# jc-bao/gym-xarm

Hardware: AMD Instinct MI355X
Metric: env steps/sec (whole node), XarmPDPickAndPlace-v0 (higher is better)
Workload: dtype f32

## Files before the change

gym_xarm_amd/build.py:

```python
import os
import shutil
import subprocess
import sys

HERE = os.path.dirname(os.path.abspath(__file__))
CSRC = os.path.join(HERE, "csrc")
LIB = os.path.join(CSRC, "libxarm_hip.so")
UNITS = ["xarm_hip.hip", "xarm_k_pnp.hip", "xarm_k_pnp_coop.hip", "xarm_k_reach.hip", "xarm_k_handover.hip", "xarm_k_handover_coop.hip",
         "xarm_k_handover2.hip", "xarm_k_stack.hip", "xarm_k_rearrange.hip", "xarm_k_render.hip", "xarm_k_her.hip", "xarm_k_norm.hip", "xarm_k_policy.hip"]
HEADERS = ["xarm_dev.h", "xarm_core.h", "xarm7_pd_model.h", "xarm_reach_core.h", "xarm7_reach_model.h", "xarm_handover_core.h", "xarm_handover2_core.h",
           "xarm_stack_core.h", "xarm_rearrange_core.h", "xarm_cubes_dev.h", "xarm_coop_core.h", "xarm_reach_coop_core.h", "xarm_handover_coop_core.h", "xarm_render_core.h",
           "xarm_render_model.h", "xarm_her_core.h", "xarm_norm_core.h", "xarm_policy_core.h"]
SOURCES = UNITS + HEADERS
UNIT_FLAGS = {"xarm_k_handover_coop.hip": ["-ffp-contract=on", "-DXC_SWEEP_COPY", "-DXC_PAD_ROWS_V1", "-DXC_PAD_SETUP_V1"], "xarm_k_norm.hip": ["-ffp-contract=off"],
              "xarm_k_policy.hip": ["-ffp-contract=off"]}
_SCHED = [] if os.environ.get("XARM_SCHED", "ilp") == "default" else ["-mllvm", "-amdgpu-sched-strategy=iterative-ilp"]
HIPCC_FLAGS = ["--offload-arch=gfx950", "-O3", "-std=c++17", "-fPIC", "-Wno-unused-value", "-fno-slp-vectorize"] + _SCHED

def find_hipcc():
    for c in (os.environ.get("HIPCC"), shutil.which("hipcc"), "/opt/rocm/bin/hipcc"):
        if c and os.path.exists(c):
            return c
    raise RuntimeError("hipcc not found (need ROCm); set HIPCC=/path/to/hipcc")


def stale():
    if not os.path.exists(LIB):
        return True
    deps = [os.path.join(CSRC, s) for s in SOURCES] + [os.path.join(os.path.dirname(HERE), "include", "xarm_hip.h")]
    t = os.path.getmtime(LIB)
    return any(os.path.getmtime(d) > t for d in deps if os.path.exists(d))


def _compile(args):
    cmd, verbose = args
    if verbose:
        print(" ".join(cmd), flush=True)
    subprocess.check_call(cmd)


def build(force=False, verbose=True, extra_flags=(), lib=LIB, jobs=None):
    from concurrent.futures import ThreadPoolExecutor
    for g in ("gen_model_header.py", "gen_render_header.py"):
        gen = os.path.join(os.path.dirname(HERE), "tools", g)
        if os.path.exists(gen):
            subprocess.check_call([sys.executable, gen], stdout=subprocess.DEVNULL)
    if not force and lib == LIB and not stale():
        return lib
    hipcc = find_hipcc()
    objdir = os.path.join(CSRC, "build" if lib == LIB else "build_" + os.path.splitext(os.path.basename(lib))[0])
    os.makedirs(objdir, exist_ok=True)
    objs, jobs_l = [], []
    for u in UNITS:
        o = os.path.join(objdir, os.path.splitext(u)[0] + ".o")
        objs.append(o)
        jobs_l.append(([hipcc] + HIPCC_FLAGS + UNIT_FLAGS.get(u, []) + list(extra_flags) + ["-c", "-o", o, os.path.join(CSRC, u)], verbose))
    with ThreadPoolExecutor(jobs or min(len(UNITS), os.cpu_count() or 1)) as ex:
        list(ex.map(_compile, jobs_l))
    _compile(([hipcc, "--offload-arch=gfx950", "-shared", "-fPIC", "-o", lib] + objs, verbose))
    return lib


def build_example(verbose=True):
    root = os.path.dirname(HERE)
    src, out = os.path.join(root, "examples", "abi_step_loop.c"), os.path.join(root, "examples", "abi_step_loop")
    if not os.path.exists(src):
        return None
    if os.path.exists(out) and os.path.getmtime(out) >= max(os.path.getmtime(src), os.path.getmtime(os.path.join(root, "include", "xarm_hip.h"))):
        return out
    rocm = os.environ.get("ROCM_PATH", "/opt/rocm")
    cmd = ["gcc", "-O2", "-std=c11", "-I", os.path.join(root, "include"), "-I", os.path.join(rocm, "include"), src,
           "-L", CSRC, "-lxarm_hip", "-L", os.path.join(rocm, "lib"), "-lamdhip64",
           "-Wl,-rpath,$ORIGIN/../gym_xarm_amd/csrc", "-Wl,-rpath," + os.path.join(rocm, "lib"), "-o", out]
    if verbose:
        print(" ".join(cmd), flush=True)
    subprocess.check_call(cmd)
    return out


if __name__ == "__main__":
    build(force="--force" in sys.argv)
    print(LIB)
```

gym_xarm_amd/csrc/xarm_coop_core.h:

```cpp
#pragma once
#include "xarm_core.h"

namespace xc {
using xk::V3; using xk::mk; using xk::dot; using xk::cross; using xk::symmul; using xk::tri; using xk::symi;
using xk::EnvState; using xk::EnvCfg; using xk::NTS; using xk::NP; using xk::clampT; using xk::xabs; using xk::xsqrt;
using xk::LDS_S; using xk::LDS_T;

constexpr int GL = 16;
constexpr int NT = 3 * NTS;
constexpr int NA1 = 14;
constexpr int NF = 3 * NP;
constexpr int NLA = 7;
constexpr int C0_T = 0, C0_F = NT, C0_N = NT + NF;
constexpr int C1_A = 0, C1_L = NA1, C1_F = NA1 + NLA, C1_N = NA1 + NLA + NF;
constexpr int C2_T = 0, C2_A = NT, C2_L = NT + NA1, C2_F = NT + NA1 + NLA, C2_N = NT + NA1 + NLA + NF;

#if defined(__HIPCC__) && !defined(XARM_HOST_BUILD)
constexpr int LVN = 1;
struct Grp { int l; };
XARM_HD int lane_of(const Grp &G, int) { return G.l; }
template <int CTRL> XARM_HD float dpp(float x) {
    return __builtin_bit_cast(float, __builtin_amdgcn_update_dpp(0, __builtin_bit_cast(int, x), CTRL, 0xf, 0xf, true));
}
#else
// ... 39 lines not shown
template <typename T> XARM_HD LV<T> lv_med3(LV<T> x, LV<T> lo, LV<T> hi) { LV<T> r; XC_LANES r.v[i_] = med3(x.v[i_], lo.v[i_], hi.v[i_]); return r; }
XARM_HD float max0(float x) { return __builtin_fmaxf(x, 0.0f); }
XARM_HD double max0(double x) { return x < 0.0 ? 0.0 : x; }
template <typename T> XARM_HD LV<T> lv_max0(LV<T> x) { LV<T> r; XC_LANES r.v[i_] = max0(x.v[i_]); return r; }
template <int L, typename T> XARM_HD void lv_commit(const Grp &G, LV<T> &dst, LV<T> src) {
    XC_LANES dst.v[i_] = lane_of(G, i_) == L ? src.v[i_] : dst.v[i_];
}
#if defined(__HIPCC__) && !defined(XARM_HOST_BUILD)
template <int L> XARM_HD LV<float> lv_bcast(LV<float> x) { LV<float> r; r.v[0] = dpp<0x150 + L>(x.v[0]); return r; }
XARM_HD float lv_allsum(LV<float> x) {
    XC_NO_CONTRACT
    float s = x.v[0];
    s += dpp<0xB1>(s);
    s += dpp<0x4E>(s);
    s += dpp<0x141>(s);
    s += dpp<0x140>(s);
    return s;
}
#else
template <int L, typename T> XARM_HD LV<T> lv_bcast(LV<T> x) { LV<T> r; XC_LANES r.v[i_] = x.v[L]; return r; }
template <typename T> XARM_HD T lv_allsum(LV<T> x) {
    T a[GL], b[GL];
    for (int i = 0; i < GL; i++) a[i] = x.v[i];
    for (int i = 0; i < GL; i++) b[i] = a[i] + a[i ^ 1];
    for (int i = 0; i < GL; i++) a[i] = b[i] + b[i ^ 2];
    for (int i = 0; i < GL; i++) b[i] = a[i] + a[(i & 8) | (7 - (i & 7))];
    for (int i = 0; i < GL; i++) a[i] = b[i] + b[15 - i];
    return a[0];
}
#endif
template <int L, typename T> XARM_HD T lv_get(LV<T> x) { return lv_bcast<L>(x).v[0]; }
#if defined(__HIPCC__) && !defined(XARM_HOST_BUILD)
XARM_HD LV<float> lv_suffix_sum(LV<float> x) {
    XC_NO_CONTRACT
    float s = x.v[0];
    s += dpp<0x101>(s);
    s += dpp<0x102>(s);
    s += dpp<0x104>(s);
    s += dpp<0x108>(s);
    LV<float> r; r.v[0] = s; return r;
}
#else
template <typename T> XARM_HD LV<T> lv_suffix_sum(LV<T> x) {
    T a[GL], b[GL];
    for (int i = 0; i < GL; i++) a[i] = x.v[i];
    for (int sh = 1; sh < GL; sh *= 2) {
        for (int i = 0; i < GL; i++) b[i] = a[i] + (i + sh < GL ? a[i + sh] : (T)0);
        for (int i = 0; i < GL; i++) a[i] = b[i];
    }
    LV<T> r; for (int i = 0; i < GL; i++) r.v[i] = a[i]; return r;
}
#endif

#if defined(__HIPCC__) && !defined(XARM_HOST_BUILD)
template <typename T> struct LV2 { xk::xf2 v; };
XARM_HD LV2<float> lv2_make(LV<float> x, LV<float> y) { LV2<float> r; r.v.x = x.v[0]; r.v.y = y.v[0]; return r; }
XARM_HD LV<float> lv2_x(LV2<float> a) { LV<float> r; r.v[0] = a.v.x; return r; }
XARM_HD LV<float> lv2_y(LV2<float> a) { LV<float> r; r.v[0] = a.v.y; return r; }
XARM_HD LV2<float> lv2_fma(LV2<float> a, LV2<float> b, LV2<float> c) { LV2<float> r; r.v = __builtin_elementwise_fma(a.v, b.v, c.v); return r; }
XARM_HD LV2<float> lv2_sub(LV2<float> a, LV2<float> b) { XC_NO_CONTRACT LV2<float> r; r.v = a.v - b.v; return r; }
XARM_HD LV2<float> lv2_mul(LV2<float> a, LV2<float> b) { XC_NO_CONTRACT LV2<float> r; r.v = a.v * b.v; return r; }
template <int L> XARM_HD void lv2_commit(const Grp &G, LV2<float> &dst, LV2<float> src) { dst.v = G.l == L ? src.v : dst.v; }
template <int L> XARM_HD LV2<float> lv2_bcast(LV2<float> x) {
    LV2<float> r;
    const long long in = __builtin_bit_cast(long long, x.v);
    const long long out = __builtin_amdgcn_update_dpp(0ll, in, 0x150 + L, 0xf, 0xf, true);
    r.v = __builtin_bit_cast(xk::xf2, out);
    return r;
}
#else
template <typename T> struct LV2 { LV<T> x, y; };
template <typename T> XARM_HD LV2<T> lv2_make(LV<T> x, LV<T> y) { LV2<T> r; r.x = x; r.y = y; return r; }
template <typename T> XARM_HD LV<T> lv2_x(LV2<T> a) { return a.x; }
template <typename T> XARM_HD LV<T> lv2_y(LV2<T> a) { return a.y; }
template <typename T> XARM_HD LV2<T> lv2_fma(LV2<T> a, LV2<T> b, LV2<T> c) { return lv2_make(lv_fma(a.x, b.x, c.x), lv_fma(a.y, b.y, c.y)); }
template <typename T> XARM_HD LV2<T> lv2_sub(LV2<T> a, LV2<T> b) { return lv2_make(lv_sub(a.x, b.x), lv_sub(a.y, b.y)); }
template <typename T> XARM_HD LV2<T> lv2_mul(LV2<T> a, LV2<T> b) { return lv2_make(lv_mul(a.x, b.x), lv_mul(a.y, b.y)); }
template <int L, typename T> XARM_HD void lv2_commit(const Grp &G, LV2<T> &dst, LV2<T> src) { lv_commit<L>(G, dst.x, src.x); lv_commit<L>(G, dst.y, src.y); }
template <int L, typename T> XARM_HD LV2<T> lv2_bcast(LV2<T> x) { return lv2_make(lv_bcast<L>(x.x), lv_bcast<L>(x.y)); }
#endif

template <typename T> XARM_HD T sel3(int k, T a, T b, T c) { return k == 0 ? a : (k == 1 ? b : c); }
template <typename T> XARM_HD T sel4(int k, T a, T b, T c, T d) { return k == 0 ? a : (k == 1 ? b : (k == 2 ? c : d)); }
template <typename T> XARM_HD V3<T> selv3(int k, V3<T> a, V3<T> b, V3<T> c) { return mk<T>(sel3(k, a.x, b.x, c.x), sel3(k, a.y, b.y, c.y), sel3(k, a.z, b.z, c.z)); }
template <typename T> XARM_HD V3<T> selv4(int k, V3<T> a, V3<T> b, V3<T> c, V3<T> d) {
    return mk<T>(sel4(k, a.x, b.x, c.x, d.x), sel4(k, a.y, b.y, c.y, d.y), sel4(k, a.z, b.z, c.z, d.z));
}

template <typename T> struct Setup {
    T Minv[45], dq[9];
    V3<T> hc1;
    V3<T> cb, vb, wb;
    T Iinv[6];
    V3<T> tr[NTS];
    T tvt[NTS], tl0[NTS];
    int tid[NTS];
    T m_vt[9], la_vt[7], la_sg[7], lf_vt[2][2], g_vt;
    LV<T> lpp[3], lpn[3], lpt1[3], lpvt, lpl0;
    bool pact[NP];
    bool pad_any, la_any;
    T pad_cfm, mu_p;
};

enum { R_J0 = 0,
       R_J1 = 6,
       R_J2A = 15,
       R_J2B = 24,
       R_J3 = 30,
       R_G = 37,
       R_L0 = 41,
       R_LO1 = 45, R_HI1 = 46,
       R_CFM = 47,
       R_N = 48 };

template <typename T> XARM_HD V3<T> tdir(int a) { return mk<T>(a == 2 ? (T)1 : (T)0, a == 1 ? (T)-1 : (T)0, a == 0 ? (T)1 : (T)0); }

template <typename T, typename Scene = xk::PnpScene>
XARM_HD void lane_rows_base(const Setup<T> &S, int l, T (&R)[R_N]) {
    const T inf = (T)3.0e38;
#pragma unroll
    for (int k = 0; k < R_N; k++) R[k] = (T)0;
    {
        const int s = l / 3, a = l - 3 * s;
        const bool own = l < NT;
        const V3<T> d = tdir<T>(a);
        const V3<T> r = selv4(s, S.tr[0], S.tr[1], S.tr[2], S.tr[3]);
        const V3<T> rd = cross(r, d);
        R[R_J0 + 0] = own ? d.x : (T)0; R[R_J0 + 1] = own ? d.y : (T)0; R[R_J0 + 2] = own ? d.z : (T)0;
        R[R_J0 + 3] = own ? rd.x : (T)0; R[R_J0 + 4] = own ? rd.y : (T)0; R[R_J0 + 5] = own ? rd.z : (T)0;
        const T vt = a == 0 ? sel4(s, S.tvt[0], S.tvt[1], S.tvt[2], S.tvt[3]) : (T)0;
        const T ju = R[R_J0 + 0] * S.vb.x + R[R_J0 + 1] * S.vb.y + R[R_J0 + 2] * S.vb.z + R[R_J0 + 3] * S.wb.x + R[R_J0 + 4] * S.wb.y + R[R_J0 + 5] * S.wb.z;
        R[R_G + 0] = own ? vt - ju : (T)0;
        R[R_L0 + 0] = (own && a == 0) ? sel4(s, S.tl0[0], S.tl0[1], S.tl0[2], S.tl0[3]) : (T)0;
    }
    {
#pragma unroll
        for (int d = 0; d < 7; d++) R[R_J1 + d] = l == d ? (T)1 : (T)0;
        R[R_J1 + 7] = (l == 7 || l == 9 || l == 13) ? (T)1 : (l == 10 ? (T)-1 : (T)0);
        R[R_J1 + 8] = (l == 8 || l == 11) ? (T)1 : ((l == 12 || l == 13) ? (T)-1 : (T)0);
        T vt = (T)0, ju = (T)0;
#pragma unroll
        for (int d = 0; d < 9; d++) { vt = l == d ? S.m_vt[d] : vt; ju += R[R_J1 + d] * S.dq[d]; }
        vt = l == 9 ? S.lf_vt[0][0] : (l == 10 ? S.lf_vt[0][1] : (l == 11 ? S.lf_vt[1][0] : (l == 12 ? S.lf_vt[1][1] : (l == 13 ? S.g_vt : vt))));
        R[R_G + 1] = l < NA1 ? vt - ju : (T)0;
        const T m_hi_arm = (T)(xm::ARM_MOTOR_FORCE * Scene::TIME_STEP), m_hi_fin = (T)(Scene::FINGER_MOTOR_FORCE * Scene::TIME_STEP);
        const T g_hi = (T)(xm::GEAR_MAX_FORCE * Scene::TIME_STEP);
        const T hi = l < 7 ? m_hi_arm : (l < 9 ? m_hi_fin : (l < 13 ? inf : (l == 13 ? g_hi : (T)0)));
        R[R_HI1] = hi;
        R[R_LO1] = (l >= 9 && l < 13) ? (T)0 : -hi;
    }
}

template <typename T, typename Lds, bool PAD, bool LA>
XARM_HD void lane_rows_extra(const Setup<T> &S, Lds lds, int l, int li, T (&R)[R_N]) {
    if (PAD) {
        const int idx = l / 3, a = l - 3 * idx;
        const bool own = l < NF;
        const int fk = idx / xm::NPAD;
        const V3<T> p = mk<T>(S.lpp[0].v[li], S.lpp[1].v[li], S.lpp[2].v[li]);
        const V3<T> n = mk<T>(S.lpn[0].v[li], S.lpn[1].v[li], S.lpn[2].v[li]);
        const V3<T> t1 = mk<T>(S.lpt1[0].v[li], S.lpt1[1].v[li], S.lpt1[2].v[li]);
        const V3<T> t2 = cross(n, t1);
        const V3<T> d = selv3(a, n, t1, t2);
        const V3<T> mo = cross(p, d);
        const V3<T> af = S.hc1 * (fk == 0 ? (T)1 : (T)-1);
        const T wf = dot(af, d);
        T ju = (T)0;
#pragma unroll
        for (int i = 0; i < 7; i++) {
            const T j = lds[LDS_S + i * 6 + 0] * mo.x + lds[LDS_S + i * 6 + 1] * mo.y + lds[LDS_S + i * 6 + 2] * mo.z +
                        lds[LDS_S + i * 6 + 3] * d.x + lds[LDS_S + i * 6 + 4] * d.y + lds[LDS_S + i * 6 + 5] * d.z;
            R[R_J2A + i] = own ? j : (T)0;
            ju += R[R_J2A + i] * S.dq[i];
        }
        R[R_J2A + 7] = (own && fk == 0) ? wf : (T)0;
        R[R_J2A + 8] = (own && fk == 1) ? wf : (T)0;
        ju += R[R_J2A + 7] * S.dq[7] + R[R_J2A + 8] * S.dq[8];
        const V3<T> rb = p - S.cb;
        const V3<T> rd = cross(rb, d);
        R[R_J2B + 0] = own ? -d.x : (T)0; R[R_J2B + 1] = own ? -d.y : (T)0; R[R_J2B + 2] = own ? -d.z : (T)0;
        R[R_J2B + 3] = own ? -rd.x : (T)0; R[R_J2B + 4] = own ? -rd.y : (T)0; R[R_J2B + 5] = own ? -rd.z : (T)0;
        ju += R[R_J2B + 0] * S.vb.x + R[R_J2B + 1] * S.vb.y + R[R_J2B + 2] * S.vb.z + R[R_J2B + 3] * S.wb.x + R[R_J2B + 4] * S.wb.y + R[R_J2B + 5] * S.wb.z;
        const T vt = a == 0 ? S.lpvt.v[li] : (T)0;
        R[R_G + 2] = own ? vt - ju : (T)0;
        R[R_L0 + 2] = (own && a == 0) ? S.lpl0.v[li] : (T)0;
        R[R_CFM] = (own && a == 0) ? S.pad_cfm : (T)0;
    }
    if (LA) {
        T vt = (T)0, ju = (T)0;
#pragma unroll
        for (int d = 0; d < 7; d++) {
            R[R_J3 + d] = l == d ? S.la_sg[d] : (T)0;
            vt = l == d ? S.la_vt[d] : vt;
            ju += R[R_J3 + d] * S.dq[d];
        }
        R[R_G + 3] = l < NLA ? vt - ju : (T)0;
    }
}

template <typename T> XARM_HD void arm_row_B(const Setup<T> &S, int r, T (&B)[9]) {
#pragma unroll
    for (int d = 0; d < 9; d++) {
        if (r < 9) B[d] = S.Minv[symi(d, r)];
        else if (r == 9) B[d] = S.Minv[symi(d, 7)];
        else if (r == 10) B[d] = -S.Minv[symi(d, 7)];
        else if (r == 11) B[d] = S.Minv[symi(d, 8)];
        else if (r == 12) B[d] = -S.Minv[symi(d, 8)];
        else if (r == 13) B[d] = S.Minv[symi(d, 7)] - S.Minv[symi(d, 8)];
        else B[d] = S.la_sg[r - NA1] * S.Minv[symi(d, r - NA1)];
    }
}
template <typename T, typename Scene = xk::PnpScene>
XARM_HD void lane_delassus_base(const Setup<T> &S, int l, const T (&R)[R_N], T (&nA0)[C0_N], T (&nA1)[C1_N], T (&invd)[4]) {
    const T imb = (T)(1.0 / Scene::OBJ_MASS);
#pragma unroll
    for (int k = 0; k < 4; k++) invd[k] = (T)0;
    T diag0 = (T)1, diag1 = (T)1;
    bool act0 = false;
#pragma unroll
    for (int s = 0; s < NTS; s++)
#pragma unroll
        for (int a = 0; a < 3; a++) {
            const int r = 3 * s + a;
            const V3<T> d = tdir<T>(a);
            const V3<T> bl = d * imb, ba = symmul(S.Iinv, cross(S.tr[s], d));
            const T a0 = R[R_J0 + 0] * bl.x + R[R_J0 + 1] * bl.y + R[R_J0 + 2] * bl.z + R[R_J0 + 3] * ba.x + R[R_J0 + 4] * ba.y + R[R_J0 + 5] * ba.z;
            nA0[C0_T + r] = -a0;
            diag0 = l == r ? a0 : diag0;
            act0 = l == r ? S.tid[s] >= 0 : act0;
        }
    invd[0] = act0 ? (T)1 / diag0 : (T)0;
#pragma unroll
    for (int r = 0; r < NA1; r++) {
        T B[9];
        arm_row_B(S, r, B);
        T a1 = (T)0;
#pragma unroll
        for (int d = 0; d < 9; d++) a1 += R[R_J1 + d] * B[d];
        nA1[C1_A + r] = -a1;
        diag1 = l == r ? a1 : diag1;
    }
    invd[1] = l < NA1 ? (T)1 / diag1 : (T)0;
}
template <typename T, bool PAD, bool LA, typename Scene = xk::PnpScene>
XARM_HD void lane_delassus_extra(const Setup<T> &S, int l, const T (&R)[R_N], T (&nA1)[C1_N], T (&nA2)[C2_N], T (&nA3)[C1_N], T (&invd)[4]) {
    const T imb = (T)(1.0 / Scene::OBJ_MASS);
    T diag3 = (T)1;
    bool act3 = false;
    if (PAD) {
#pragma unroll
        for (int s = 0; s < NTS; s++)
#pragma unroll
            for (int a = 0; a < 3; a++) {
                const int r = 3 * s + a;
                const V3<T> d = tdir<T>(a);
                const V3<T> bl = d * imb, ba = symmul(S.Iinv, cross(S.tr[s], d));
                nA2[C2_T + r] = -(R[R_J2B + 0] * bl.x + R[R_J2B + 1] * bl.y + R[R_J2B + 2] * bl.z + R[R_J2B + 3] * ba.x + R[R_J2B + 4] * ba.y + R[R_J2B + 5] * ba.z);
            }
    }
#pragma unroll
    for (int r = 0; r < NA1 + NLA; r++) {
        if (!LA && r >= NA1) continue;
        T B[9];
        arm_row_B(S, r, B);
        T a1 = (T)0, a2 = (T)0, a3 = (T)0;
#pragma unroll
        for (int d = 0; d < 9; d++) {
            if (r >= NA1) a1 += R[R_J1 + d] * B[d];
            if (PAD) a2 += R[R_J2A + d] * B[d];
            if (LA && d < 7) a3 += R[R_J3 + d] * B[d];
        }
        const int c1 = r < NA1 ? C1_A + r : C1_L + (r - NA1);
        if (r >= NA1) nA1[c1] = -a1;
        if (PAD) nA2[(r < NA1 ? C2_A + r : C2_L + (r - NA1))] = -a2;
        if (LA) nA3[c1] = -a3;
        if (r >= NA1) { diag3 = l == r - NA1 ? a3 : diag3; act3 = l == r - NA1 ? S.la_sg[r - NA1] != (T)0 : act3; }
    }
    if (LA) invd[3] = act3 ? (T)1 / diag3 : (T)0;
}

template <typename T> struct Sweep {
    LV<T> g[4], lam[4], invd[4];
    LV<T> lo1, hi1;
    LV<T> nA0[C0_N], nA1[C1_N], nA2[C2_N], nA3[C1_N];
#ifndef XC_PAD_SETUP_V1
    LV2<T> AF01[NF];
    LV<T> AF2[NF];
#endif
};

template <typename T, typename Scene = xk::PnpScene>
XARM_HD void pad_minv_jt(const Setup<T> &S, const LV<T> (&J)[R_G], LV<T> (&Ba)[9], LV<T> (&Bb)[6]) {
    const T imb = (T)(1.0 / Scene::OBJ_MASS);
#pragma unroll
    for (int q = 0; q < 9; q++) {
        LV<T> s = lv_scale(J[R_J2A + 0], S.Minv[symi(q, 0)]);
#pragma unroll
        for (int i = 1; i < 9; i++) s = lv_fmas(J[R_J2A + i], S.Minv[symi(q, i)], s);
        Ba[q] = s;
    }
#pragma unroll
    for (int d = 0; d < 3; d++) Bb[d] = lv_scale(J[R_J2B + d], imb);
    Bb[3] = lv_fmas(J[R_J2B + 5], S.Iinv[2], lv_fmas(J[R_J2B + 4], S.Iinv[1], lv_scale(J[R_J2B + 3], S.Iinv[0])));
    Bb[4] = lv_fmas(J[R_J2B + 5], S.Iinv[4], lv_fmas(J[R_J2B + 4], S.Iinv[3], lv_scale(J[R_J2B + 3], S.Iinv[1])));
    Bb[5] = lv_fmas(J[R_J2B + 5], S.Iinv[5], lv_fmas(J[R_J2B + 4], S.Iinv[4], lv_scale(J[R_J2B + 3], S.Iinv[2])));
}
#if defined(__HIPCC__) && !defined(XARM_HOST_BUILD) && !defined(XC_PAD_SETUP_V1)
#define XC_DPP_BC(r) " row_newbcast:" #r " row_mask:0xf bank_mask:0xf bound_ctrl:1\n\t"
#define XC_PAD_DOTS(r, a0, a1, a2)                                                                           \
    asm("s_nop 1\n\t"                                                                                        \
        "v_mul_f32_dpp %[x2], %[p0], %[f0]" XC_DPP_BC(r) "v_mul_f32_dpp %[x1], %[p0], %[s0]" XC_DPP_BC(r) "v_mul_f32_dpp %[x0], %[o0], %[t0]" XC_DPP_BC(r)    \
        "v_fmac_f32_dpp %[x2], %[p1], %[f1]" XC_DPP_BC(r) "v_fmac_f32_dpp %[x1], %[p1], %[s1]" XC_DPP_BC(r) "v_fmac_f32_dpp %[x0], %[o1], %[t1]" XC_DPP_BC(r) \
        "v_fmac_f32_dpp %[x2], %[p2], %[f2]" XC_DPP_BC(r) "v_fmac_f32_dpp %[x1], %[p2], %[s2]" XC_DPP_BC(r) "v_fmac_f32_dpp %[x0], %[o2], %[t2]" XC_DPP_BC(r) \
        "v_fmac_f32_dpp %[x2], %[p3], %[f3]" XC_DPP_BC(r) "v_fmac_f32_dpp %[x1], %[p3], %[s3]" XC_DPP_BC(r) "v_fmac_f32_dpp %[x0], %[o3], %[t3]" XC_DPP_BC(r) \
        "v_fmac_f32_dpp %[x2], %[p4], %[f4]" XC_DPP_BC(r) "v_fmac_f32_dpp %[x1], %[p4], %[s4]" XC_DPP_BC(r) "v_fmac_f32_dpp %[x0], %[o4], %[t4]" XC_DPP_BC(r) \
        "v_fmac_f32_dpp %[x2], %[p5], %[f5]" XC_DPP_BC(r) "v_fmac_f32_dpp %[x1], %[p5], %[s5]" XC_DPP_BC(r) "v_fmac_f32_dpp %[x0], %[o5], %[t5]" XC_DPP_BC(r) \
        "v_fmac_f32_dpp %[x2], %[p6], %[f6]" XC_DPP_BC(r) "v_fmac_f32_dpp %[x1], %[p6], %[s6]" XC_DPP_BC(r)                                                    \
        "v_fmac_f32_dpp %[x2], %[p7], %[f7]" XC_DPP_BC(r) "v_fmac_f32_dpp %[x1], %[p7], %[s7]" XC_DPP_BC(r)                                                    \
        "v_fmac_f32_dpp %[x2], %[p8], %[f8]" XC_DPP_BC(r) "v_fmac_f32_dpp %[x1], %[p8], %[s8]" XC_DPP_BC(r)                                                    \
        "v_fmac_f32_dpp %[x2], %[o0], %[g0]" XC_DPP_BC(r) "v_fmac_f32_dpp %[x2], %[o1], %[g1]" XC_DPP_BC(r) "v_fmac_f32_dpp %[x2], %[o2], %[g2]" XC_DPP_BC(r) \
        "v_fmac_f32_dpp %[x2], %[o3], %[g3]" XC_DPP_BC(r) "v_fmac_f32_dpp %[x2], %[o4], %[g4]" XC_DPP_BC(r) "v_fmac_f32_dpp %[x2], %[o5], %[g5]" XC_DPP_BC(r) \
        : [x0] "=&v"(a0.v[0]), [x1] "=&v"(a1.v[0]), [x2] "=&v"(a2.v[0])                                      \
        : [p0] "v"(Ba[0].v[0]), [p1] "v"(Ba[1].v[0]), [p2] "v"(Ba[2].v[0]), [p3] "v"(Ba[3].v[0]), [p4] "v"(Ba[4].v[0]), [p5] "v"(Ba[5].v[0]),                 \
          [p6] "v"(Ba[6].v[0]), [p7] "v"(Ba[7].v[0]), [p8] "v"(Ba[8].v[0]),                                  \
          [o0] "v"(Bb[0].v[0]), [o1] "v"(Bb[1].v[0]), [o2] "v"(Bb[2].v[0]), [o3] "v"(Bb[3].v[0]), [o4] "v"(Bb[4].v[0]), [o5] "v"(Bb[5].v[0]),                 \
          [t0] "v"(J[R_J0 + 0].v[0]), [t1] "v"(J[R_J0 + 1].v[0]), [t2] "v"(J[R_J0 + 2].v[0]), [t3] "v"(J[R_J0 + 3].v[0]), [t4] "v"(J[R_J0 + 4].v[0]),         \
          [t5] "v"(J[R_J0 + 5].v[0]),                                                                        \
          [s0] "v"(J[R_J1 + 0].v[0]), [s1] "v"(J[R_J1 + 1].v[0]), [s2] "v"(J[R_J1 + 2].v[0]), [s3] "v"(J[R_J1 + 3].v[0]), [s4] "v"(J[R_J1 + 4].v[0]),         \
          [s5] "v"(J[R_J1 + 5].v[0]), [s6] "v"(J[R_J1 + 6].v[0]), [s7] "v"(J[R_J1 + 7].v[0]), [s8] "v"(J[R_J1 + 8].v[0]),                                     \
          [f0] "v"(J[R_J2A + 0].v[0]), [f1] "v"(J[R_J2A + 1].v[0]), [f2] "v"(J[R_J2A + 2].v[0]), [f3] "v"(J[R_J2A + 3].v[0]), [f4] "v"(J[R_J2A + 4].v[0]),    \
          [f5] "v"(J[R_J2A + 5].v[0]), [f6] "v"(J[R_J2A + 6].v[0]), [f7] "v"(J[R_J2A + 7].v[0]), [f8] "v"(J[R_J2A + 8].v[0]),                                 \
          [g0] "v"(J[R_J2B + 0].v[0]), [g1] "v"(J[R_J2B + 1].v[0]), [g2] "v"(J[R_J2B + 2].v[0]), [g3] "v"(J[R_J2B + 3].v[0]), [g4] "v"(J[R_J2B + 4].v[0]),    \
          [g5] "v"(J[R_J2B + 5].v[0]))
#endif
template <typename T, bool LA, typename Scene = xk::PnpScene>
XARM_HD void pad_columns(const Grp &G, const Setup<T> &S, const LV<T> (&J)[R_G], LV<T> cfm, Sweep<T> &W, const bool (&padw)[NP]) {
    LV<T> Ba[9], Bb[6];
    pad_minv_jt<T, Scene>(S, J, Ba, Bb);
#ifndef XC_PAD_SETUP_V1
#ifndef XC_PAD_DOTS
#define XC_PAD_DOTS(r, a0, a1, a2)                                                                           \
    {                                                                                                        \
        LV<T> ca[9], cb[6];                                                                                  \
        _Pragma("unroll") for (int q = 0; q < 9; q++) ca[q] = lv_bcast<r>(Ba[q]);                            \
        _Pragma("unroll") for (int d = 0; d < 6; d++) cb[d] = lv_bcast<r>(Bb[d]);                            \
        a0 = lv_mul(J[R_J0], cb[0]); a1 = lv_mul(J[R_J1], ca[0]); a2 = lv_mul(J[R_J2A], ca[0]);              \
        _Pragma("unroll") for (int d = 1; d < 6; d++) a0 = lv_fma(J[R_J0 + d], cb[d], a0);                   \
        _Pragma("unroll") for (int q = 1; q < 9; q++) { a1 = lv_fma(J[R_J1 + q], ca[q], a1); a2 = lv_fma(J[R_J2A + q], ca[q], a2); } \
        _Pragma("unroll") for (int d = 0; d < 6; d++) a2 = lv_fma(J[R_J2B + d], cb[d], a2);                  \
    }
#endif
    LV<T> dg = lv_mul(J[R_J2A], Ba[0]);
#pragma unroll
    for (int q = 1; q < 9; q++) dg = lv_fma(J[R_J2A + q], Ba[q], dg);
#pragma unroll
    for (int d = 0; d < 6; d++) dg = lv_fma(J[R_J2B + d], Bb[d], dg);
    W.invd[2] = lv_rcp_pads(G, lv_add(dg, cfm), S.pact);
    const LV2<T> invd01 = lv2_make(W.invd[0], W.invd[1]);
#define XC_PAD_COL(r)                                                                                        \
    if (padw[(r) / 3]) {                                                                                     \
        LV<T> a0, a1, a2;                                                                                    \
        XC_PAD_DOTS(r, a0, a1, a2);                                                                          \
        LV<T> diag = a2;                                                                                     \
        lv_commit<r>(G, diag, lv_add(a2, cfm));  \
        W.nA0[C0_F + r] = lv_neg(a0);                                                                        \
        W.nA1[C1_F + r] = lv_neg(a1);                                                                        \
        W.nA2[C2_F + r] = lv_neg(diag);                                                                      \
// ... 404 lines not shown
                Li[tri(r, c)] = s * rd[r];
            }
        }
#pragma unroll
        for (int r = 0; r < 9; r++)
#pragma unroll
            for (int c = 0; c <= r; c++) {
                T s = (T)0;
#pragma unroll
                for (int k = r; k < 9; k++) s += Li[tri(k, r)] * Li[tri(k, c)];
                Minv[tri(r, c)] = s;
            }
    }
#pragma unroll
    for (int r = 0; r < 9; r++) {
        T s = (T)0;
#pragma unroll
        for (int c = 0; c < 9; c++) s += Minv[symi(r, c)] * tau[c];
        A.dq[r] = qd_in[r] + dt * s;
    }
#pragma unroll
    for (int i = 0; i < 7; i++) {
        lds[LDS_S + i * 6 + 0] = S[i].w.x; lds[LDS_S + i * 6 + 1] = S[i].w.y; lds[LDS_S + i * 6 + 2] = S[i].w.z;
        lds[LDS_S + i * 6 + 3] = S[i].v.x; lds[LDS_S + i * 6 + 4] = S[i].v.y; lds[LDS_S + i * 6 + 5] = S[i].v.z;
    }
    XARM_LDS_FENCE();
}

template <typename T, typename Lds, typename Scene = xk::PnpScene>
XARM_HD void substep_setup(const Grp &G, const ArmLane<T> &C, EnvState<T> &st, const T (&qt)[9], const T dt, Lds lds, Setup<T> &S, const int arm = 0) {
    const T idt = (T)1 / dt;
    xk::ArmDyn<T> AD;
    arm_dynamics_coop<T, Lds, Scene>(G, C, st.q, st.qd, dt, lds, AD, arm);
#pragma unroll
    for (int k = 0; k < 45; k++) S.Minv[k] = AD.Minv[k];
#pragma unroll
    for (int k = 0; k < 9; k++) S.dq[k] = AD.dq[k];
    S.hc1 = AD.hc1;
    const V3<T> hc0 = AD.hc0, hc1 = AD.hc1, hc2 = AD.hc2;
    V3<T> b0, b1, b2;
    {
        const T x = st.bq[0], y = st.bq[1], z = st.bq[2], w = st.bq[3];
        b0 = mk<T>((T)1 - (T)2 * (y * y + z * z), (T)2 * (x * y + z * w), (T)2 * (x * z - y * w));
        b1 = mk<T>((T)2 * (x * y - z * w), (T)1 - (T)2 * (x * x + z * z), (T)2 * (y * z + x * w));
        b2 = mk<T>((T)2 * (x * z + y * w), (T)2 * (y * z - x * w), (T)1 - (T)2 * (x * x + y * y));
    }
    const V3<T> cb = mk<T>(st.bp[0], st.bp[1], st.bp[2]);
    S.cb = cb;
    const T hx = (T)Scene::OBJ_HX, hy = (T)Scene::OBJ_HY, hz = (T)Scene::OBJ_HZ;
    const T Ibx = (T)(Scene::OBJ_MASS / 3.0 * (Scene::OBJ_HY * Scene::OBJ_HY + Scene::OBJ_HZ * Scene::OBJ_HZ));
    const T Iby = (T)(Scene::OBJ_MASS / 3.0 * (Scene::OBJ_HX * Scene::OBJ_HX + Scene::OBJ_HZ * Scene::OBJ_HZ));
    const T Ibz = (T)(Scene::OBJ_MASS / 3.0 * (Scene::OBJ_HX * Scene::OBJ_HX + Scene::OBJ_HY * Scene::OBJ_HY));
    {
        const T ix = (T)1 / Ibx, iy = (T)1 / Iby, iz = (T)1 / Ibz;
        S.Iinv[0] = b0.x * b0.x * ix + b1.x * b1.x * iy + b2.x * b2.x * iz;
        S.Iinv[1] = b0.x * b0.y * ix + b1.x * b1.y * iy + b2.x * b2.y * iz;
        S.Iinv[2] = b0.x * b0.z * ix + b1.x * b1.z * iy + b2.x * b2.z * iz;
        S.Iinv[3] = b0.y * b0.y * ix + b1.y * b1.y * iy + b2.y * b2.y * iz;
        S.Iinv[4] = b0.y * b0.z * ix + b1.y * b1.z * iy + b2.y * b2.z * iz;
        S.Iinv[5] = b0.z * b0.z * ix + b1.z * b1.z * iy + b2.z * b2.z * iz;
    }
    V3<T> vb = mk<T>(st.bv[0], st.bv[1], st.bv[2]), wb = mk<T>(st.bw[0], st.bw[1], st.bw[2]);
    {
        const V3<T> wl = mk<T>(dot(b0, wb), dot(b1, wb), dot(b2, wb));
        const V3<T> iw = mk<T>(Ibx * wl.x, Iby * wl.y, Ibz * wl.z);
        const V3<T> f = cross(wl, iw) * dt;
        const T J00 = Ibx, J01 = dt * (-wl.z * Iby + iw.z), J02 = dt * (wl.y * Ibz - iw.y);
        const T J10 = dt * (wl.z * Ibx - iw.z), J11 = Iby, J12 = dt * (-wl.x * Ibz + iw.x);
        const T J20 = dt * (-wl.y * Ibx + iw.y), J21 = dt * (wl.x * Iby - iw.x), J22 = Ibz;
        const T c00 = J11 * J22 - J12 * J21, c01 = J12 * J20 - J10 * J22, c02 = J10 * J21 - J11 * J20;
        const T id = (T)1 / (J00 * c00 + J01 * c01 + J02 * c02);
        const V3<T> x = mk<T>((f.x * c00 + f.y * (J02 * J21 - J01 * J22) + f.z * (J01 * J12 - J02 * J11)) * id,
                              (f.x * c01 + f.y * (J00 * J22 - J02 * J20) + f.z * (J02 * J10 - J00 * J12)) * id,
                              (f.x * c02 + f.y * (J01 * J20 - J00 * J21) + f.z * (J00 * J11 - J01 * J10)) * id);
        const V3<T> wn = wl - x;
        wb = b0 * wn.x + b1 * wn.y + b2 * wn.z;
        vb.z -= dt * (T)xm::GRAVITY;
        vb = vb * (T)Scene::LIN_DAMP_FACTOR;
        wb = wb * (T)Scene::ANG_DAMP_FACTOR;
    }
    S.vb = vb; S.wb = wb;
#pragma unroll
    for (int s = 0; s < NTS; s++) { S.tr[s] = mk<T>(0, 0, 0); S.tvt[s] = (T)0; S.tl0[s] = (T)0; S.tid[s] = -1; }
    {
        int cnt = 0;
#pragma unroll
        for (int i = 0; i < 8; i++) {
            const V3<T> r = b0 * ((i & 1) ? hx : -hx) + b1 * ((i & 2) ? hy : -hy) + b2 * ((i & 4) ? hz : -hz);
            const V3<T> p = cb + r;
            T hsup;
            const bool sup = Scene::template support<T>(p, hsup);
            const T dist = p.z - hsup;
            const bool act = dist < (T)xm::SOLVER_MARGIN && sup && cnt < NTS;
            const T vt = dist < (T)0 ? -(T)xm::CONTACT_ERP * dist * idt : -dist * idt;
            const T l0 = (T)xm::WARMSTART * st.lam_t[i];
#pragma unroll
            for (int s = 0; s < NTS; s++) {
                const bool put = act && cnt == s;
                S.tr[s] = xk::selv(put, r, S.tr[s]);
                S.tvt[s] = put ? vt : S.tvt[s];
                S.tl0[s] = put ? l0 : S.tl0[s];
                S.tid[s] = put ? i : S.tid[s];
            }
            cnt += act ? 1 : 0;
        }
        if constexpr (Scene::HAS_STAND) {
            V3<T> sp[4];
            T sd[4];
            Scene::template stand_points<T>(st.goal, cb, b0, b1, b2, sp, sd);
#pragma unroll
            for (int v = 0; v < 4; v++) {
                const T dist = sd[v];
                const bool act = dist < (T)xm::SOLVER_MARGIN && dist > (T)Scene::STAND_MIN_GAP && cnt < NTS;
                const V3<T> r = sp[v] - cb;
                const T vt = dist < (T)0 ? -(T)xm::CONTACT_ERP * dist * idt : -dist * idt;
#pragma unroll
                for (int s = 0; s < NTS; s++) {
                    const bool put = act && cnt == s;
                    S.tr[s] = xk::selv(put, r, S.tr[s]);
                    S.tvt[s] = put ? vt : S.tvt[s];
                    S.tl0[s] = put ? (T)0 : S.tl0[s];
                    S.tid[s] = put ? 8 + v : S.tid[s];
                }
                cnt += act ? 1 : 0;
            }
        }
    }
#pragma unroll
    for (int i = 0; i < 9; i++) S.m_vt[i] = (T)xm::MOTOR_KP * (qt[i] - st.q[i]) * idt + (T)(1.0 - xm::MOTOR_KD) * S.dq[i];
    bool la_any = false;
#pragma unroll
    for (int i = 0; i < 7; i++) {
        const T g0 = st.q[i] - (T)xm::LOWER[i], g1 = (T)xm::UPPER[i] - st.q[i];
        const bool lo = g0 < (T)xm::LIMIT_WINDOW, hi = g1 < (T)xm::LIMIT_WINDOW;
        const T g = lo ? g0 : g1;
        S.la_sg[i] = lo ? (T)1 : (hi ? (T)-1 : (T)0);
        S.la_vt[i] = g < (T)0 ? -(T)xm::GLOBAL_ERP * g * idt : -g * idt;
        la_any = la_any || S.la_sg[i] != (T)0;
    }
    S.la_any = la_any;
#pragma unroll
    for (int k = 0; k < 2; k++) {
        const T g0 = st.q[7 + k] - (T)xm::LOWER[7 + k], g1 = (T)xm::UPPER[7 + k] - st.q[7 + k];
        S.lf_vt[k][0] = g0 < (T)0 ? -(T)xm::GLOBAL_ERP * g0 * idt : -g0 * idt;
        S.lf_vt[k][1] = g1 < (T)0 ? -(T)xm::GLOBAL_ERP * g1 * idt : -g1 * idt;
    }
    S.g_vt = -(T)(xm::GEAR_ERP * xm::GLOBAL_ERP) * (st.q[7] - st.q[8]) * idt;
    const T pad_denom = dt * (T)xm::FINGER_CONTACT_STIFFNESS + (T)(xm::FINGER_CONTACT_DAMPING + xm::OBJECT_CONTACT_DAMPING);
    const T pad_erp = dt * (T)xm::FINGER_CONTACT_STIFFNESS / pad_denom;
    S.pad_cfm = ((T)1 / pad_denom) * idt;
    static_assert(xm::NPAD == 2 && NP == 4, "pad dealing below");
    LV<T> actf, tchf;
    XC_LANES {
        const int l = lane_of(G, i_);
        const int idx = l / 3 < NP ? l / 3 : NP - 1;
        const int fk = idx >> 1, j = idx & 1;
        const T sg = fk == 0 ? (T)1 : (T)-1;
        const T pc0 = j == 0 ? (T)xm::PAD_C[0][0] : (T)xm::PAD_C[1][0], pc1 = j == 0 ? (T)xm::PAD_C[0][1] : (T)xm::PAD_C[1][1];
        const T pc2 = j == 0 ? (T)xm::PAD_C[0][2] : (T)xm::PAD_C[1][2];
        const V3<T> c = xk::selv(fk == 0, AD.fo[0], AD.fo[1]) + hc0 * pc0 + hc1 * (sg * pc1) + hc2 * pc2;
        const V3<T> d = c - cb;
        const V3<T> cl = mk<T>(dot(b0, d), dot(b1, d), dot(b2, d));
        const V3<T> ql = mk<T>(clampT(cl.x, -hx, hx), clampT(cl.y, -hy, hy), clampT(cl.z, -hz, hz));
        const V3<T> dl = cl - ql;
        const T d2 = dot(dl, dl);
        V3<T> nl, pl;
        T dist;
        if (d2 > (T)1e-12) {
            const T len = xsqrt(d2);
            nl = dl * ((T)1 / len);
            dist = len - (T)xm::PAD_RADIUS;
            pl = ql;
        } else {
            const T px = hx - xabs(cl.x), py = hy - xabs(cl.y), pz = hz - xabs(cl.z);
            int k = 0;
            T best = px;
            if (py < best) { best = py; k = 1; }
            if (pz < best) { best = pz; k = 2; }
            const T clk = k == 0 ? cl.x : (k == 1 ? cl.y : cl.z);
            const T s1 = clk < (T)0 ? (T)-1 : (T)1;
            nl = mk<T>(k == 0 ? s1 : (T)0, k == 1 ? s1 : (T)0, k == 2 ? s1 : (T)0);
            dist = -best - (T)xm::PAD_RADIUS;
            pl = mk<T>(k == 0 ? s1 * hx : cl.x, k == 1 ? s1 * hy : cl.y, k == 2 ? s1 * hz : cl.z);
        }
        const bool act = dist < (T)xm::SOLVER_MARGIN;
        actf.v[i_] = act ? (T)1 : (T)0;
        tchf.v[i_] = dist < (T)xm::CONTACT_MARGIN ? (T)1 : (T)0;
        const V3<T> pn = b0 * nl.x + b1 * nl.y + b2 * nl.z;
        const V3<T> pp = cb + b0 * pl.x + b1 * pl.y + b2 * pl.z;
        const V3<T> pt1 = xk::plane_space(pn);
        S.lpn[0].v[i_] = pn.x; S.lpn[1].v[i_] = pn.y; S.lpn[2].v[i_] = pn.z;
        S.lpp[0].v[i_] = pp.x; S.lpp[1].v[i_] = pp.y; S.lpp[2].v[i_] = pp.z;
        S.lpt1[0].v[i_] = pt1.x; S.lpt1[1].v[i_] = pt1.y; S.lpt1[2].v[i_] = pt1.z;
        S.lpvt.v[i_] = dist < (T)0 ? -pad_erp * dist * idt : -dist * idt;
        S.lpl0.v[i_] = act ? (T)xm::WARMSTART * sel4(idx, st.lam_p[0], st.lam_p[1], st.lam_p[2], st.lam_p[3]) : (T)0;
    }
    S.pact[0] = lv_get<0>(actf) != (T)0; S.pact[1] = lv_get<3>(actf) != (T)0;
    S.pact[2] = lv_get<6>(actf) != (T)0; S.pact[3] = lv_get<9>(actf) != (T)0;
    S.pad_any = S.pact[0] || S.pact[1] || S.pact[2] || S.pact[3];
    const bool touch_f[2] = {lv_get<0>(tchf) != (T)0 || lv_get<3>(tchf) != (T)0, lv_get<6>(tchf) != (T)0 || lv_get<9>(tchf) != (T)0};
    S.mu_p = (T)xm::MU_OBJECT * (st.mug > (T)0.5 ? (T)xm::MU_FINGER_GRASP : (T)xm::MU_FINGER);
    st.touch = (touch_f[0] && touch_f[1]) ? (T)1 : (T)0;
}

template <typename T, typename Scene = xk::PnpScene>
XARM_HD void build_base(const Grp &G, const Setup<T> &S, Sweep<T> &W, LV<T> (&J)[R_G]) {
    XC_LANES {
        const int l = lane_of(G, i_);
        T R[R_N], a0[C0_N], a1[C1_N], iv[4];
        lane_rows_base<T, Scene>(S, l, R);
        lane_delassus_base<T, Scene>(S, l, R, a0, a1, iv);
#pragma unroll
        for (int k = 0; k < R_J2A; k++) J[k].v[i_] = R[k];
#pragma unroll
        for (int k = 0; k < 2; k++) { W.g[k].v[i_] = R[R_G + k]; W.lam[k].v[i_] = R[R_L0 + k]; W.invd[k].v[i_] = iv[k]; }
        W.lo1.v[i_] = R[R_LO1]; W.hi1.v[i_] = R[R_HI1];
#pragma unroll
        for (int k = 0; k < NT; k++) W.nA0[C0_T + k].v[i_] = a0[C0_T + k];
#pragma unroll
        for (int k = 0; k < NA1; k++) W.nA1[C1_A + k].v[i_] = a1[C1_A + k];
    }
}
template <typename T, typename Lds, bool PAD, bool LA, typename Scene = xk::PnpScene>
XARM_HD void build_extra(const Grp &G, const Setup<T> &S, Lds lds, Sweep<T> &W, LV<T> (&J)[R_G], LV<T> &cfm) {
    XC_LANES {
        const int l = lane_of(G, i_);
        T R[R_N], a1[C1_N], a2[C2_N], a3[C1_N], iv[4];
#pragma unroll
        for (int k = 0; k < R_N; k++) R[k] = k < R_J2A ? J[k].v[i_] : (T)0;
#pragma unroll
        for (int k = 0; k < C1_N; k++) a1[k] = a3[k] = (T)0;
#pragma unroll
        for (int k = 0; k < C2_N; k++) a2[k] = (T)0;
#pragma unroll
        for (int k = 0; k < 4; k++) iv[k] = (T)0;
        lane_rows_extra<T, Lds, PAD, LA>(S, lds, l, i_, R);
        lane_delassus_extra<T, PAD, LA, Scene>(S, l, R, a1, a2, a3, iv);
#pragma unroll
        for (int k = R_J2A; k < R_G; k++) J[k].v[i_] = R[k];
#pragma unroll
        for (int k = 2; k < 4; k++) { W.g[k].v[i_] = R[R_G + k]; W.lam[k].v[i_] = R[R_L0 + k]; W.invd[k].v[i_] = iv[k]; }
        cfm.v[i_] = R[R_CFM];
#pragma unroll
        for (int k = C1_L; k < C1_N; k++) W.nA1[k].v[i_] = a1[k];
#pragma unroll
        for (int k = NT; k < C0_N; k++) W.nA0[k].v[i_] = (T)0;
#pragma unroll
        for (int k = 0; k < C1_N; k++) W.nA3[k].v[i_] = a3[k];
#pragma unroll
        for (int k = 0; k < C2_N; k++) W.nA2[k].v[i_] = a2[k];
    }
}

template <typename T, typename Lds, bool PAD, bool LA>
XARM_HD void solve(const Grp &G, const Setup<T> &S, Lds lds, EnvState<T> &st, Sweep<T> &W, LV<T> (&J)[R_G], T (&tau)[15]) {
    LV<T> cfm = lv_fill((T)0);
    if (PAD || LA) build_extra<T, Lds, PAD, LA>(G, S, lds, W, J, cfm);
    bool padw[NP];
#pragma unroll
#if defined(XC_FORCE_FULL) || defined(XC_FORCE_PADW)
    for (int p = 0; p < NP; p++) padw[p] = PAD;
#else
    for (int p = 0; p < NP; p++) padw[p] = PAD && XARM_ANY_X(S.pact[p]);
#endif
    if (PAD) pad_columns<T, LA>(G, S, J, cfm, W, padw);
    apply_warm_start<T, PAD, LA>(W, padw);
    const T mu_t = (T)(xm::MU_OBJECT * xm::MU_TABLE);
    sweep_all<T, PAD, LA>(G, W, mu_t, S.mu_p, padw);
#pragma unroll
    for (int d = 0; d < 9; d++) {
        LV<T> c = lv_mul(J[R_J1 + d], W.lam[1]);
        if (PAD) c = lv_fma(J[R_J2A + d], W.lam[2], c);
        if (LA && d < 7) c = lv_fma(J[R_J3 + d], W.lam[3], c);
        tau[d] = lv_allsum(c);
    }
#pragma unroll
    for (int d = 0; d < 6; d++) {
        LV<T> c = lv_mul(J[R_J0 + d], W.lam[0]);
        if (PAD) c = lv_fma(J[R_J2B + d], W.lam[2], c);
        tau[9 + d] = lv_allsum(c);
    }
    const T lt[NTS] = {lv_get<0>(W.lam[0]), lv_get<3>(W.lam[0]), lv_get<6>(W.lam[0]), lv_get<9>(W.lam[0])};
#pragma unroll
    for (int i = 0; i < 8; i++) {
        T l = (T)0;
#pragma unroll
        for (int s = 0; s < NTS; s++) l = S.tid[s] == i ? lt[s] : l;
        st.lam_t[i] = l;
        st.lam_p[i] = (T)0;
    }
    if (PAD) {
        st.lam_p[0] = lv_get<0>(W.lam[2]); st.lam_p[1] = lv_get<3>(W.lam[2]);
        st.lam_p[2] = lv_get<6>(W.lam[2]); st.lam_p[3] = lv_get<9>(W.lam[2]);
    }
}

template <typename T, typename Lds>
XARM_HD void substep(const Grp &G, const ArmLane<T> &C, EnvState<T> &st, const T (&qt)[9], const T dt, Lds lds) {
    Setup<T> S;
    substep_setup<T, Lds>(G, C, st, qt, dt, lds, S);
    XARM_LDS_FENCE();
    T tau[15];
    Sweep<T> W;
    LV<T> J[R_G];
    build_base<T>(G, S, W, J);
#ifdef XC_FORCE_FULL
    const bool pad = true, la = true;
#elif defined(XC_FORCE_PAD)
    const bool pad = true, la = XARM_ANY_X(S.la_any);
#elif defined(XC_FORCE_LA)
    const bool pad = XARM_ANY_X(S.pad_any), la = true;
#else
    const bool pad = XARM_ANY_X(S.pad_any), la = XARM_ANY_X(S.la_any);
#endif
    if (pad) {
        if (la) solve<T, Lds, true, true>(G, S, lds, st, W, J, tau);
        else solve<T, Lds, true, false>(G, S, lds, st, W, J, tau);
    } else {
        if (la) solve<T, Lds, false, true>(G, S, lds, st, W, J, tau);
        else solve<T, Lds, false, false>(G, S, lds, st, W, J, tau);
    }
    const T imb = (T)(1.0 / xk::PnpScene::OBJ_MASS);
#pragma unroll
    for (int r = 0; r < 9; r++) {
        T s = S.dq[r];
#pragma unroll
        for (int c = 0; c < 9; c++) s += S.Minv[symi(r, c)] * tau[c];
        st.qd[r] = s;
        st.q[r] += dt * s;
    }
    const V3<T> vb = S.vb + mk<T>(tau[9], tau[10], tau[11]) * imb;
    const V3<T> wb = S.wb + symmul(S.Iinv, mk<T>(tau[12], tau[13], tau[14]));
    st.bp[0] += dt * vb.x; st.bp[1] += dt * vb.y; st.bp[2] += dt * vb.z;
    {
        const T idt = (T)1 / dt;
        T ang = xsqrt(dot(wb, wb));
        if (ang * dt > (T)0.7853981633974483) ang = (T)0.7853981633974483 * idt;
        T sw, cw;
        xk::xsincos((T)0.5 * ang * dt, sw, cw);
        const T k = ang < (T)0.001 ? (T)0.5 * dt - dt * dt * dt * (T)0.020833333333 * ang * ang : sw / ang;
        const V3<T> ax = wb * k;
        const T x = st.bq[0], y = st.bq[1], z = st.bq[2], w0 = st.bq[3];
        const T nx = cw * x + ax.x * w0 + ax.y * z - ax.z * y;
        const T ny = cw * y + ax.y * w0 + ax.z * x - ax.x * z;
        const T nz = cw * z + ax.z * w0 + ax.x * y - ax.y * x;
        const T nw = cw * w0 - ax.x * x - ax.y * y - ax.z * z;
        const T inv = (T)1 / xsqrt(nx * nx + ny * ny + nz * nz + nw * nw);
        st.bq[0] = nx * inv; st.bq[1] = ny * inv; st.bq[2] = nz * inv; st.bq[3] = nw * inv;
    }
    st.bv[0] = vb.x; st.bv[1] = vb.y; st.bv[2] = vb.z;
    st.bw[0] = wb.x; st.bw[1] = wb.y; st.bw[2] = wb.z;
}

template <typename T, typename Lds> XARM_HD void sim_tick(const Grp &G, const ArmLane<T> &C, EnvState<T> &st, const T (&qt)[9], Lds lds) {
    const T dt = (T)(xm::PNP_TIME_STEP / xm::PNP_N_SUBSTEPS);
#pragma unroll 1
    for (int k = 0; k < xm::PNP_N_SUBSTEPS; k++) substep<T, Lds>(G, C, st, qt, dt, lds);
}

template <typename T, typename Lds> XARM_HD void env_reset(const Grp &G, const EnvCfg &cfg, int64_t env, EnvState<T> &st, Lds lds) {
    const ArmLane<T> C = arm_lane_consts<T>(G);
    T qt[9];
    const int64_t episode = (int64_t)st.episode + 1;
    const V3<T> start = mk<T>((T)xm::PNP_START_GRIPPER_POS[0], (T)xm::PNP_START_GRIPPER_POS[1], (T)xm::PNP_START_GRIPPER_POS[2]);
#pragma unroll 1
    for (int k = 0; k < xm::PNP_RESET_TICKS + 1; k++) {
        if (k < xm::PNP_RESET_TICKS) {
            xk::ik_solve(st.q, start, qt);
            qt[7] = qt[8] = (T)xm::PNP_RESET_FINGER_TARGET;
        } else {
// ... 34 lines not shown
```

Baseline: 18.54 million.

## Restructure table-contact setup with corner bitmask and cross-lane column build

Adds a second setup path, enabled by default except in the handover-coop unit. It selects active box corners with a bitmask and ctz instead of a serial counter, and uses a branchless 8-way select for warm-start lambdas. Table-contact Delassus columns and diagonal inverses are now built cooperatively across lanes with DPP broadcasts of the angular terms, replacing the per-lane NTS-by-row loops. The lam_t writeback loop is also trimmed using the ordering invariant. This aims to cut per-lane setup ALU and register pressure, at the cost of extra cross-lane broadcasts and a reliance on tid ordering.

Result: no change. 18.67 million, median of 6 (+0.7%).

```diff
diff --git a/gym_xarm_amd/build.py b/gym_xarm_amd/build.py
--- a/gym_xarm_amd/build.py
+++ b/gym_xarm_amd/build.py
@@ -12,7 +12,7 @@
            "xarm_stack_core.h", "xarm_rearrange_core.h", "xarm_cubes_dev.h", "xarm_coop_core.h", "xarm_reach_coop_core.h", "xarm_handover_coop_core.h", "xarm_render_core.h",
            "xarm_render_model.h", "xarm_her_core.h", "xarm_norm_core.h", "xarm_policy_core.h"]
 SOURCES = UNITS + HEADERS
-UNIT_FLAGS = {"xarm_k_handover_coop.hip": ["-ffp-contract=on", "-DXC_SWEEP_COPY", "-DXC_PAD_ROWS_V1", "-DXC_PAD_SETUP_V1"], "xarm_k_norm.hip": ["-ffp-contract=off"],
+UNIT_FLAGS = {"xarm_k_handover_coop.hip": ["-ffp-contract=on", "-DXC_SWEEP_COPY", "-DXC_PAD_ROWS_V1", "-DXC_PAD_SETUP_V1", "-DXC_SETUP_V2_OFF"], "xarm_k_norm.hip": ["-ffp-contract=off"],
               "xarm_k_policy.hip": ["-ffp-contract=off"]}
 _SCHED = [] if os.environ.get("XARM_SCHED", "ilp") == "default" else ["-mllvm", "-amdgpu-sched-strategy=iterative-ilp"]
 HIPCC_FLAGS = ["--offload-arch=gfx950", "-O3", "-std=c++17", "-fPIC", "-Wno-unused-value", "-fno-slp-vectorize"] + _SCHED
diff --git a/gym_xarm_amd/csrc/xarm_coop_core.h b/gym_xarm_amd/csrc/xarm_coop_core.h
--- a/gym_xarm_amd/csrc/xarm_coop_core.h
+++ b/gym_xarm_amd/csrc/xarm_coop_core.h
@@ -145,6 +145,12 @@
 
 template <typename T> XARM_HD T sel3(int k, T a, T b, T c) { return k == 0 ? a : (k == 1 ? b : c); }
 template <typename T> XARM_HD T sel4(int k, T a, T b, T c, T d) { return k == 0 ? a : (k == 1 ? b : (k == 2 ? c : d)); }
+template <typename T> XARM_HD T sel8(int k, T a0, T a1, T a2, T a3, T a4, T a5, T a6, T a7) {
+    const bool k0 = k & 1, k1 = k & 2, k2 = k & 4;
+    const T b0 = k0 ? a1 : a0, b1 = k0 ? a3 : a2, b2 = k0 ? a5 : a4, b3 = k0 ? a7 : a6;
+    const T c0 = k1 ? b1 : b0, c1 = k1 ? b3 : b2;
+    return k2 ? c1 : c0;
+}
 template <typename T> XARM_HD V3<T> selv3(int k, V3<T> a, V3<T> b, V3<T> c) { return mk<T>(sel3(k, a.x, b.x, c.x), sel3(k, a.y, b.y, c.y), sel3(k, a.z, b.z, c.z)); }
 template <typename T> XARM_HD V3<T> selv4(int k, V3<T> a, V3<T> b, V3<T> c, V3<T> d) {
     return mk<T>(sel4(k, a.x, b.x, c.x, d.x), sel4(k, a.y, b.y, c.y, d.y), sel4(k, a.z, b.z, c.z, d.z));
@@ -278,7 +284,9 @@
     const T imb = (T)(1.0 / Scene::OBJ_MASS);
 #pragma unroll
     for (int k = 0; k < 4; k++) invd[k] = (T)0;
-    T diag0 = (T)1, diag1 = (T)1;
+    T diag1 = (T)1;
+#ifdef XC_SETUP_V2_OFF
+    T diag0 = (T)1;
     bool act0 = false;
 #pragma unroll
     for (int s = 0; s < NTS; s++)
@@ -293,6 +301,9 @@
             act0 = l == r ? S.tid[s] >= 0 : act0;
         }
     invd[0] = act0 ? (T)1 / diag0 : (T)0;
+#else
+    (void)imb; (void)nA0;
+#endif
 #pragma unroll
     for (int r = 0; r < NA1; r++) {
         T B[9];
@@ -310,6 +321,7 @@
     const T imb = (T)(1.0 / Scene::OBJ_MASS);
     T diag3 = (T)1;
     bool act3 = false;
+#ifdef XC_SETUP_V2_OFF
     if (PAD) {
 #pragma unroll
         for (int s = 0; s < NTS; s++)
@@ -321,6 +333,9 @@
                 nA2[C2_T + r] = -(R[R_J2B + 0] * bl.x + R[R_J2B + 1] * bl.y + R[R_J2B + 2] * bl.z + R[R_J2B + 3] * ba.x + R[R_J2B + 4] * ba.y + R[R_J2B + 5] * ba.z);
             }
     }
+#else
+    (void)imb;
+#endif
 #pragma unroll
     for (int r = 0; r < NA1 + NLA; r++) {
         if (!LA && r >= NA1) continue;
@@ -346,6 +361,9 @@
     LV<T> g[4], lam[4], invd[4];
     LV<T> lo1, hi1;
     LV<T> nA0[C0_N], nA1[C1_N], nA2[C2_N], nA3[C1_N];
+#ifndef XC_SETUP_V2_OFF
+    LV<T> tba[3];
+#endif
 #ifndef XC_PAD_SETUP_V1
     LV2<T> AF01[NF];
     LV<T> AF2[NF];
@@ -916,7 +934,40 @@
     S.vb = vb; S.wb = wb;
 #pragma unroll
     for (int s = 0; s < NTS; s++) { S.tr[s] = mk<T>(0, 0, 0); S.tvt[s] = (T)0; S.tl0[s] = (T)0; S.tid[s] = -1; }
-    {
+#ifndef XC_SETUP_V2_OFF
+    constexpr bool CORNERS_BY_MASK = !Scene::HAS_STAND;
+#else
+    constexpr bool CORNERS_BY_MASK = false;
+#endif
+    if constexpr (CORNERS_BY_MASK) {
+        unsigned mask = 0;
+#pragma unroll
+        for (int i = 0; i < 8; i++) {
+            const V3<T> r = b0 * ((i & 1) ? hx : -hx) + b1 * ((i & 2) ? hy : -hy) + b2 * ((i & 4) ? hz : -hz);
+            const V3<T> p = cb + r;
+            T hsup;
+            const bool sup = Scene::template support<T>(p, hsup);
+            const T dist = p.z - hsup;
+            mask |= (dist < (T)xm::SOLVER_MARGIN && sup) ? 1u << i : 0u;
+        }
+#pragma unroll
+        for (int s = 0; s < NTS; s++) {
+            const bool put = mask != 0;
+            const int i = put ? __builtin_ctz(mask) : 0;
+            mask &= mask - 1;
+            const V3<T> r = b0 * ((i & 1) ? hx : -hx) + b1 * ((i & 2) ? hy : -hy) + b2 * ((i & 4) ? hz : -hz);
+            const V3<T> p = cb + r;
+            T hsup;
+            Scene::template support<T>(p, hsup);
+            const T dist = p.z - hsup;
+            const T vt = dist < (T)0 ? -(T)xm::CONTACT_ERP * dist * idt : -dist * idt;
+            const T l0 = (T)xm::WARMSTART * sel8(i, st.lam_t[0], st.lam_t[1], st.lam_t[2], st.lam_t[3], st.lam_t[4], st.lam_t[5], st.lam_t[6], st.lam_t[7]);
+            S.tr[s] = xk::selv(put, r, S.tr[s]);
+            S.tvt[s] = put ? vt : S.tvt[s];
+            S.tl0[s] = put ? l0 : S.tl0[s];
+            S.tid[s] = put ? i : S.tid[s];
+        }
+    } else {
         int cnt = 0;
 #pragma unroll
         for (int i = 0; i < 8; i++) {
@@ -1037,6 +1088,46 @@
     st.touch = (touch_f[0] && touch_f[1]) ? (T)1 : (T)0;
 }
 
+#ifndef XC_SETUP_V2_OFF
+template <int JB, typename T> XARM_HD void table_cols(const LV<T> (&J)[R_G], const LV<T> (&tba)[3], const T imb, LV<T> *dst) {
+    LV<T> x[NT];
+#pragma unroll
+    for (int r = 0; r < NT; r++) {
+        const V3<T> bl = tdir<T>(r % 3) * imb;
+        XC_LANES x[r].v[i_] = J[JB + 0].v[i_] * bl.x + J[JB + 1].v[i_] * bl.y + J[JB + 2].v[i_] * bl.z;
+    }
+#define XC_TC(r)                                                                                             \
+    {                                                                                                        \
+        const LV<T> c0 = lv_bcast<r>(tba[0]), c1 = lv_bcast<r>(tba[1]), c2 = lv_bcast<r>(tba[2]);            \
+        XC_LANES x[r].v[i_] = x[r].v[i_] + J[JB + 3].v[i_] * c0.v[i_] + J[JB + 4].v[i_] * c1.v[i_] + J[JB + 5].v[i_] * c2.v[i_]; \
+    }
+    XC_TC(0) XC_TC(1) XC_TC(2) XC_TC(3) XC_TC(4) XC_TC(5) XC_TC(6) XC_TC(7) XC_TC(8) XC_TC(9) XC_TC(10) XC_TC(11)
+#undef XC_TC
+#pragma unroll
+    for (int r = 0; r < NT; r++) XC_LANES dst[r].v[i_] = -x[r].v[i_];
+}
+template <typename T, typename Scene = xk::PnpScene>
+XARM_HD void table_columns(const Grp &G, const Setup<T> &S, const LV<T> (&J)[R_G], Sweep<T> &W) {
+    const T imb = (T)(1.0 / Scene::OBJ_MASS);
+    XC_LANES {
+        const int l = lane_of(G, i_);
+        const int s = l / 3, a = l - 3 * s;
+        const V3<T> bl = tdir<T>(a) * imb;
+        const V3<T> ba = symmul(S.Iinv, mk<T>(J[R_J0 + 3].v[i_], J[R_J0 + 4].v[i_], J[R_J0 + 5].v[i_]));
+        W.tba[0].v[i_] = ba.x; W.tba[1].v[i_] = ba.y; W.tba[2].v[i_] = ba.z;
+        const T dg = J[R_J0 + 0].v[i_] * bl.x + J[R_J0 + 1].v[i_] * bl.y + J[R_J0 + 2].v[i_] * bl.z +
+                     J[R_J0 + 3].v[i_] * ba.x + J[R_J0 + 4].v[i_] * ba.y + J[R_J0 + 5].v[i_] * ba.z;
+        const bool act = l < NT && sel4(s, S.tid[0], S.tid[1], S.tid[2], S.tid[3]) >= 0;
+        W.invd[0].v[i_] = act ? (T)1 / dg : (T)0;
+    }
+    table_cols<R_J0>(J, W.tba, imb, &W.nA0[C0_T]);
+}
+template <typename T, typename Scene = xk::PnpScene>
+XARM_HD void table_columns_pad(const LV<T> (&J)[R_G], Sweep<T> &W) {
+    table_cols<R_J2B>(J, W.tba, (T)(1.0 / Scene::OBJ_MASS), &W.nA2[C2_T]);
+}
+#endif
+
 template <typename T, typename Scene = xk::PnpScene>
 XARM_HD void build_base(const Grp &G, const Setup<T> &S, Sweep<T> &W, LV<T> (&J)[R_G]) {
     XC_LANES {
@@ -1049,11 +1140,16 @@
 #pragma unroll
         for (int k = 0; k < 2; k++) { W.g[k].v[i_] = R[R_G + k]; W.lam[k].v[i_] = R[R_L0 + k]; W.invd[k].v[i_] = iv[k]; }
         W.lo1.v[i_] = R[R_LO1]; W.hi1.v[i_] = R[R_HI1];
+#ifdef XC_SETUP_V2_OFF
 #pragma unroll
         for (int k = 0; k < NT; k++) W.nA0[C0_T + k].v[i_] = a0[C0_T + k];
+#endif
 #pragma unroll
         for (int k = 0; k < NA1; k++) W.nA1[C1_A + k].v[i_] = a1[C1_A + k];
     }
+#ifndef XC_SETUP_V2_OFF
+    table_columns<T, Scene>(G, S, J, W);
+#endif
 }
 template <typename T, typename Lds, bool PAD, bool LA, typename Scene = xk::PnpScene>
 XARM_HD void build_extra(const Grp &G, const Setup<T> &S, Lds lds, Sweep<T> &W, LV<T> (&J)[R_G], LV<T> &cfm) {
@@ -1084,6 +1180,9 @@
 #pragma unroll
         for (int k = 0; k < C2_N; k++) W.nA2[k].v[i_] = a2[k];
     }
+#ifndef XC_SETUP_V2_OFF
+    if (PAD) table_columns_pad<T, Scene>(J, W);
+#endif
 }
 
 template <typename T, typename Lds, bool PAD, bool LA>
@@ -1119,7 +1218,11 @@
     for (int i = 0; i < 8; i++) {
         T l = (T)0;
 #pragma unroll
+#ifndef XC_SETUP_V2_OFF
+        for (int s = 0; s < NTS && s <= i; s++) l = S.tid[s] == i ? lt[s] : l;
+#else
         for (int s = 0; s < NTS; s++) l = S.tid[s] == i ? lt[s] : l;
+#endif
         st.lam_t[i] = l;
         st.lam_p[i] = (T)0;
     }
```
